# yanyan-li/PlanarSLAM

Measured on AMD Instinct MI355X. Metric: RGB-D frames/sec (extract+match+pose-opt) @640x480; 1->8-GPU batch scaling, higher is better.
Workload: dtype u8/f64

## Files before the change

planarslam_amd/csrc/lsd.hip:

```cpp
#include "common.h"
#include "wave_ops.h"
#include "lsd_nfa.h"
#include "isort.h"

namespace planar {
namespace lsd {

constexpr double LSD_PI = 3.14159265358979323846;
constexpr double M_3_2_PI = 3 * LSD_PI / 2, M_2__PI = 2 * LSD_PI;
constexpr float NOTDEF_F = -1024.0f;
constexpr double DEG_TO_RADS = LSD_PI / 180;
constexpr double RELATIVE_ERROR_FACTOR = 100.0;
constexpr int N_BINS = 1024;
constexpr int MAX_SEGS = 2048;
constexpr int MAX_RECTS = 4096;
constexpr int RING = 512;
constexpr int USED_LDS_BITS = 32768;

struct Plan {
    int W, H, w, h;
    int taps7[7], taps5[5];
    double rho, prec, p, log_nt, density_th, log_eps;
    int min_reg_size;
    size_t off_blur7, off_blur5, off_dx, off_dy, off_ang, off_g2, off_pix, off_seed, off_ord, off_ordr, off_gused, off_tmp, off_reg, off_valid, off_sortr, off_sortb, off_heapj, off_segs, off_kl, off_rects, off_res, off_est, frame_bytes;
    const double* lgamma_tab;
    double p_log[12], p1_log[12], p_log10[12];
    double gaussCoefL[21], gaussCoefG[63];
};

struct Misc { uint32_t g2max; int n_ord; int n_seg; int n_kl; int status; int n_regions; int n_grown_px; int n_rect; long long t[8]; int sort_counts[2]; int heap_n; int sort_kv; int sort_prefix; int pad_; float imp_T; int imp_done; int imp_redo; int imp_full; };

__device__ __forceinline__ float fast_atan2_deg(float y, float x) {
    const float scale = (float)(180 / 3.1415926535897932384626433832795);
    const float p1 = 0.9997878412794807f * scale, p3 = -0.3258083974640975f * scale;
    const float p5 = 0.1555786518463281f * scale, p7 = -0.04432655554792128f * scale;
    const float ax = fabsf(x), ay = fabsf(y);
    float a, c, c2;
    if (ax >= ay) {
        c = ay / (ax + 2.220446049250313e-16f);
        c2 = c * c;
        a = (((p7 * c2 + p5) * c2 + p3) * c2 + p1) * c;
    } else {
        c = ax / (ay + 2.220446049250313e-16f);
        c2 = c * c;
        a = 90.f - (((p7 * c2 + p5) * c2 + p3) * c2 + p1) * c;
    }
    if (x < 0) a = 180.f - a;
    if (y < 0) a = 360.f - a;
    return a;
}

__device__ __forceinline__ int reflect101(int p, int n) {
    if (n == 1) return 0;
    while (p < 0 || p >= n) p = p < 0 ? -p : 2 * n - 2 - p;
    return p;
}

template <int KS>
__global__ __launch_bounds__(256) void lsd_gauss(const uint8_t* __restrict__ src, int pitch, int64_t src_stride, int W, int H,
                                                 const int* __restrict__ taps_g, uint8_t* __restrict__ ws, size_t frame_bytes, size_t off_dst, int B) {
    constexpr int R = KS / 2, TW = 64, TH = 16;
    __shared__ uint8_t s_in[TH + 2 * R][TW + 2 * R];
    __shared__ uint16_t s_h[TH + 2 * R][TW];
    int taps[KS];
    for (int i = 0; i < KS; i++) taps[i] = taps_g[i];
    const int tiles_x = (W + TW - 1) / TW, tiles_y = (H + TH - 1) / TH, tid = threadIdx.x;
    int b, tile;
    xcd_frame_block(tiles_x * tiles_y, B, b, tile);
    const int x0 = (tile % tiles_x) * TW, y0 = (tile / tiles_x) * TH;
    const uint8_t* S = src + (int64_t)b * src_stride;
    for (int i = tid; i < (TH + 2 * R) * (TW + 2 * R); i += 256) {
        const int r = i / (TW + 2 * R), c = i % (TW + 2 * R);
        s_in[r][c] = S[(int64_t)reflect101(y0 + r - R, H) * pitch + reflect101(x0 + c - R, W)];
    }
    __syncthreads();
    for (int i = tid; i < (TH + 2 * R) * TW; i += 256) {
        const int r = i / TW, c = i % TW;
        uint32_t s = 0;
        for (int k = 0; k < KS; k++) s += (uint32_t)taps[k] * s_in[r][c + k];
        s_h[r][c] = (uint16_t)min(s, 65535u);
    }
    __syncthreads();
    uint8_t* D = ws + (size_t)b * frame_bytes + off_dst;
    for (int i = tid; i < TH * TW; i += 256) {
        const int r = i / TW, c = i % TW;
        const int x = x0 + c, y = y0 + r;
        if (x >= W || y >= H) continue;
        uint32_t s = 0;
        for (int k = 0; k < KS; k++) s += (uint32_t)taps[k] * s_h[r + k][c];
        D[(size_t)y * W + x] = (uint8_t)min((s + 32768u) >> 16, 255u);
    }
}

__global__ __launch_bounds__(256) void lsd_gauss75(const uint8_t* __restrict__ src, int pitch, int64_t src_stride, int W, int H, const int* __restrict__ taps_g,
                                                   uint8_t* __restrict__ ws, size_t frame_bytes, size_t off7, size_t off5, int B) {
    constexpr int TW = 64, TH = 16, R = 3, NR = TH + 2 * R, NWD = TW / 4 + 2;
    __shared__ uint32_t s_in[NR][NWD + 1];
    __shared__ __attribute__((aligned(8))) uint16_t s_h7[NR][TW + 4], s_h5[NR][TW + 4];
    int t7[7], t5[5];
    for (int i = 0; i < 7; i++) t7[i] = taps_g[i];
    for (int i = 0; i < 5; i++) t5[i] = taps_g[8 + i];
    const int tiles_x = (W + TW - 1) / TW, tiles_y = (H + TH - 1) / TH, tid = threadIdx.x;
    int b, tile;
    xcd_frame_block(tiles_x * tiles_y, B, b, tile);
    const int x0 = (tile % tiles_x) * TW, y0 = (tile / tiles_x) * TH;
    const uint8_t* S = src + (int64_t)b * src_stride;
    for (int i = tid; i < NR * NWD; i += 256) {
        const int r = i / NWD, wq = i - r * NWD;
        const uint8_t* row = S + (int64_t)reflect101(y0 + r - R, H) * pitch;
        const int xb = x0 - 4 + 4 * wq;
        uint32_t v;
        if (xb >= 0 && xb + 3 < W) v = *(const uint32_t*)(row + xb);
        else v = (uint32_t)row[reflect101(xb, W)] | ((uint32_t)row[reflect101(xb + 1, W)] << 8) | ((uint32_t)row[reflect101(xb + 2, W)] << 16) | ((uint32_t)row[reflect101(xb + 3, W)] << 24);
        s_in[r][wq] = v;
    }
    __syncthreads();
    for (int i = tid; i < NR * (TW / 4); i += 256) {
        const int r = i / (TW / 4), q = i - r * (TW / 4);
        const uint32_t w0 = s_in[r][q], w1 = s_in[r][q + 1], w2 = s_in[r][q + 2];
        uint32_t px[12];
#pragma unroll
        for (int k = 0; k < 4; k++) { px[k] = (w0 >> (8 * k)) & 0xffu; px[4 + k] = (w1 >> (8 * k)) & 0xffu; px[8 + k] = (w2 >> (8 * k)) & 0xffu; }
        uint32_t h7[4], h5[4];
#pragma unroll
        for (int o = 0; o < 4; o++) {
            uint32_t a = 0, c = 0;
#pragma unroll
            for (int k = 0; k < 7; k++) a += (uint32_t)t7[k] * px[o + 1 + k];
#pragma unroll
            for (int k = 0; k < 5; k++) c += (uint32_t)t5[k] * px[o + 2 + k];
            h7[o] = min(a, 65535u); h5[o] = min(c, 65535u);
        }
        *(uint2*)&s_h7[r][4 * q] = make_uint2(h7[0] | (h7[1] << 16), h7[2] | (h7[3] << 16));
        *(uint2*)&s_h5[r][4 * q] = make_uint2(h5[0] | (h5[1] << 16), h5[2] | (h5[3] << 16));
    }
    __syncthreads();
    {
        const int r = tid >> 4, q = tid & 15;
        const int x = x0 + 4 * q, y = y0 + r;
        if (x < W && y < H) {
            uint32_t a[4] = {0, 0, 0, 0}, c[4] = {0, 0, 0, 0};
#pragma unroll
            for (int k = 0; k < 7; k++) {
                const uint2 v = *(const uint2*)&s_h7[r + k][4 * q];
                a[0] += (uint32_t)t7[k] * (v.x & 0xffffu); a[1] += (uint32_t)t7[k] * (v.x >> 16); a[2] += (uint32_t)t7[k] * (v.y & 0xffffu); a[3] += (uint32_t)t7[k] * (v.y >> 16);
            }
#pragma unroll
            for (int k = 0; k < 5; k++) {
                const uint2 v = *(const uint2*)&s_h5[r + 1 + k][4 * q];
                c[0] += (uint32_t)t5[k] * (v.x & 0xffffu); c[1] += (uint32_t)t5[k] * (v.x >> 16); c[2] += (uint32_t)t5[k] * (v.y & 0xffffu); c[3] += (uint32_t)t5[k] * (v.y >> 16);
            }
            uint32_t o7 = 0, o5 = 0;
#pragma unroll
            for (int o = 0; o < 4; o++) { o7 |= min((a[o] + 32768u) >> 16, 255u) << (8 * o); o5 |= min((c[o] + 32768u) >> 16, 255u) << (8 * o); }
            uint8_t* F = ws + (size_t)b * frame_bytes;
            *(uint32_t*)(F + off7 + (size_t)y * W + x) = o7;
            *(uint32_t*)(F + off5 + (size_t)y * W + x) = o5;
        }
    }
}

struct Coef { int ofs, c0, c1; };

__device__ __forceinline__ int scaled_px(const uint8_t* __restrict__ B7, int W, const Coef& cx, const Coef& cy) {
    const uint8_t* r0 = B7 + (size_t)cy.ofs * W + cx.ofs;
    const uint8_t* r1 = r0 + W;
    const uint32_t h0 = min((uint32_t)cx.c0 * r0[0] + (uint32_t)cx.c1 * r0[1], 65535u);
    const uint32_t h1 = min((uint32_t)cx.c0 * r1[0] + (uint32_t)cx.c1 * r1[1], 65535u);
    const uint32_t v = h0 * (uint32_t)cy.c0 + h1 * (uint32_t)cy.c1;
    return (int)min((v + 32768u) >> 16, 255u);
}

__device__ __forceinline__ float2 seed_cos_sin(float deg) {
    const double a = (double)deg * DEG_TO_RADS;
    return make_float2((float)cos(a), (float)sin(a));
}

__global__ __launch_bounds__(256) void lsd_grad(const Plan* __restrict__ plan, const Coef* __restrict__ cxs, const Coef* __restrict__ cys,
                                                uint8_t* __restrict__ ws, Misc* __restrict__ miscs) {
    __shared__ uint8_t s_px[5][68];
    const Plan& P = *plan;
    const int b = blockIdx.z;
    const int x0 = blockIdx.x * 64, y0 = blockIdx.y * 4;
    uint8_t* F = ws + (size_t)b * P.frame_bytes;
    const uint8_t* B7 = F + P.off_blur7;
    for (int i = threadIdx.x; i < 5 * 65; i += 256) {
        const int r = i / 65, c = i - r * 65;
        const int xs = min(x0 + c, P.w - 1), ys = min(y0 + r, P.h - 1);
        s_px[r][c] = (uint8_t)scaled_px(B7, P.W, cxs[xs], cys[ys]);
    }
    __syncthreads();
    const int lx = threadIdx.x & 63, ly = threadIdx.x >> 6;
    const int x = x0 + lx, y = y0 + ly;
    if (x >= P.w || y >= P.h) return;
    float* ang = (float*)(F + P.off_ang);
    uint32_t* g2a = (uint32_t*)(F + P.off_g2);
    float4* pix4 = (float4*)(F + P.off_pix);
    Misc* misc = miscs + b;
    const size_t o = (size_t)y * P.w + x;
    if (x >= P.w - 1 || y >= P.h - 1) { ang[o] = NOTDEF_F; g2a[o] = 0; pix4[o] = make_float4(NOTDEF_F, 0.f, 0.f, 0.f); return; }
    const int s00 = s_px[ly][lx], s10 = s_px[ly][lx + 1], s01 = s_px[ly + 1][lx], s11 = s_px[ly + 1][lx + 1];
    const int DA = s11 - s00, BC = s10 - s01;
    const int gx = DA + BC, gy = DA - BC;
    const int g2 = gx * gx + gy * gy;
    const double norm = sqrt(g2 / 4.0);
    g2a[o] = (uint32_t)g2;
    if (norm <= P.rho) { ang[o] = NOTDEF_F; pix4[o] = make_float4(NOTDEF_F, 0.f, 0.f, 0.f); }
    else {
        const float deg = fast_atan2_deg((float)gx, (float)(-gy));
        ang[o] = deg;
        const double a = (double)deg * DEG_TO_RADS;
        const float af = (float)a;
        pix4[o] = make_float4(deg, (float)cos((double)af), (float)sin((double)af), 0.f);
        atomicMax(&misc->g2max, (uint32_t)g2);
    }
}

template <int NW>
__device__ inline int block_exscan(int v, int* wsum, int* total) {
    const int lane = threadIdx.x & 63, w = threadIdx.x >> 6;
    int inc = v;
    for (int o = 1; o < 64; o <<= 1) { const int t = __shfl_up(inc, o, 64); if (lane >= o) inc += t; }
    __syncthreads();
    if (lane == 63) wsum[w] = inc;
    __syncthreads();
    int base = 0, tot = 0;
    for (int i = 0; i < NW; i++) { if (i < w) base += wsum[i]; tot += wsum[i]; }
    *total = tot;
    return base + inc - v;
}

__device__ __forceinline__ void wave_sync();
__device__ __forceinline__ void lds_sync();
#ifndef PLANAR_WIDE_T
#define PLANAR_WIDE_T 1024
#endif
constexpr int SORT_T = PLANAR_WIDE_T, SORT_LT = 256, SORT_E = 23, SORT_SHIFT = 20, SORT_R = 64;
constexpr int SORT_HJOBS = 1024, SORT_HCAP = 8192, SORT_HY = 2;
using SortLds = isort::LdsLayout<SORT_LT, SORT_E>;
using SortGl = isort::GlobalLayout<SORT_T>;

__global__ __launch_bounds__(SORT_T) void lsd_sort_global(const Plan* __restrict__ plan, uint8_t* __restrict__ ws, Misc* __restrict__ miscs, int rows_cap, int rows_long) {
    extern __shared__ __align__(16) uint8_t sort_lds[];
    __shared__ isort::Range s_init;
    const Plan& P = *plan;
    const int b = blockIdx.x, tid = threadIdx.x, lane = tid & 63;
    uint8_t* F = ws + (size_t)b * P.frame_bytes;
    const uint32_t* g2a = (const uint32_t*)(F + P.off_g2);
    uint32_t* arr = (uint32_t*)(F + P.off_tmp);
    unsigned long long* vb = (unsigned long long*)(F + P.off_valid);
    Misc* misc = miscs + b;
    const int w1 = P.w - 1, h1 = P.h - 1, n = w1 * h1, npix = P.w * P.h;
    const double max_grad = misc->g2max ? sqrt(misc->g2max / 4.0) : -1.0;
    const double bin_coef = (max_grad > 0) ? double(N_BINS - 1) / max_grad : 0;
    const long long ts0 = __builtin_readcyclecounter();
    __shared__ unsigned int s_kv, s_prefix;
    if (tid == 0) { s_kv = 0u; s_prefix = 0u; }
    __syncthreads();
    uint32_t kv = 0;
    for (int p0 = tid - lane; p0 < npix; p0 += SORT_T) {
        const int pix = p0 + lane, y = pix / P.w, x = pix - y * P.w;
        const bool in = pix < npix && x < w1 && y < h1;
        bool valid = false;
        if (in) {
            const double norm = sqrt(g2a[pix] / 4.0);
            const int bin = int(norm * bin_coef);
            arr[pix - y] = ((uint32_t)(N_BINS - 1 - bin) << SORT_SHIFT) | (uint32_t)pix;
            valid = !(norm <= P.rho);
            if (valid) kv = max(kv, (uint32_t)(N_BINS - 1 - bin));
        }
        const unsigned long long m = __ballot(valid);
        if (lane == 0) vb[p0 >> 6] = m;
    }
    kv = (uint32_t)planar::wave_max_f64((double)kv);
    if (lane == 0) atomicMax(&s_kv, kv);
    __syncthreads();
    kv = s_kv;
    int cnt = 0;
    for (int p0 = tid - lane; p0 < npix; p0 += SORT_T) {
        const int pix = p0 + lane, y = pix / P.w, x = pix - y * P.w;
        if (pix < npix && x < w1 && y < h1) cnt += ((arr[pix - y] >> SORT_SHIFT) <= kv) ? 1 : 0;
    }
    cnt = planar::wave_sum_i32(cnt);
    if (lane == 0) atomicAdd(&s_prefix, (unsigned int)cnt);
    if (tid == 0) s_init = isort::Range{0, n, isort::depth_limit(n)};
    __threadfence_block();
    __syncthreads();
    if (tid == 0) { misc->sort_kv = (int)kv; misc->sort_prefix = (int)s_prefix; }
    const isort::HeapSink HS{(isort::HeapJob*)(F + P.off_heapj), &misc->heap_n, SORT_HJOBS};
    isort::global_tier<SORT_SHIFT, SORT_T>(arr, &s_init, 1, SortLds::N, 64, (isort::Range*)(F + P.off_sortr), (isort::Block*)(F + P.off_sortb), isort::G_FMAX,
                                           misc->sort_counts, sort_lds, rows_cap, HS, &misc->status, kv,
                                           rows_long, (uint32_t*)(F + P.off_ord), n / 2 + 1);
    if (tid == 0) misc->t[5] = __builtin_readcyclecounter() - ts0;
}

__global__ __launch_bounds__(SORT_LT, 4) void lsd_sort_lds(const Plan* __restrict__ plan, uint8_t* __restrict__ ws, Misc* __restrict__ miscs) {
    extern __shared__ __align__(16) uint8_t sort_lds[];
    const Plan& P = *plan;
    const int b = blockIdx.x;
    uint8_t* F = ws + (size_t)b * P.frame_bytes;
    Misc* misc = miscs + b;
    const isort::Range* ranges = (const isort::Range*)(F + P.off_sortr);
    const isort::Block* blocks = (const isort::Block*)(F + P.off_sortb);
    const int nb = misc->sort_counts[1];
    const isort::HeapSink HS{(isort::HeapJob*)(F + P.off_heapj), &misc->heap_n, SORT_HJOBS};
    const long long ts0 = __builtin_readcyclecounter();
    for (int k = blockIdx.y; k < nb; k += gridDim.y) {
        const isort::Block K = blocks[k];
        isort::lds_tier<SORT_SHIFT, SORT_LT, SORT_E>((uint32_t*)(F + P.off_tmp), ranges + K.r0, K.nr, K.f, K.l, sort_lds, HS, &misc->status, (uint32_t)misc->sort_kv);
    }
    if (threadIdx.x == 0 && blockIdx.y == 0) misc->t[6] = __builtin_readcyclecounter() - ts0;
}

__global__ __launch_bounds__(64) void lsd_sort_heap(const Plan* __restrict__ plan, uint8_t* __restrict__ ws, Misc* __restrict__ miscs) {
    extern __shared__ __align__(16) uint8_t sort_lds[];
    const Plan& P = *plan;
    uint8_t* F = ws + (size_t)blockIdx.x * P.frame_bytes;
    const int nj = min(miscs[blockIdx.x].heap_n, SORT_HJOBS);
    if (nj) isort::heap_jobs<SORT_SHIFT>((uint32_t*)(F + P.off_tmp), (const isort::HeapJob*)(F + P.off_heapj), nj, blockIdx.y, gridDim.y, (uint32_t*)sort_lds, SORT_HCAP, 0, 1 << 30);
}

__global__ __launch_bounds__(SORT_T) void lsd_sort_compact(const Plan* __restrict__ plan, uint8_t* __restrict__ ws, Misc* __restrict__ miscs) {
    __shared__ int s_cnt[SORT_T / 64];
    const Plan& P = *plan;
    const int b = blockIdx.x, tid = threadIdx.x, lane = tid & 63, wave = tid >> 6;
    uint8_t* F = ws + (size_t)b * P.frame_bytes;
    const uint32_t* arr = (const uint32_t*)(F + P.off_tmp);
    const unsigned long long* vb = (const unsigned long long*)(F + P.off_valid);
    uint32_t* ord = (uint32_t*)(F + P.off_ord);
    uint32_t* ordr = (uint32_t*)(F + P.off_ordr);
    float* pixw = (float*)(F + P.off_pix);
    Misc* misc = miscs + b;
    const int n = min((P.w - 1) * (P.h - 1), misc->sort_prefix);
    const long long ts0 = __builtin_readcyclecounter();
    constexpr int NW = SORT_T / 64, U = 4;
    const int seg = ((n + NW - 1) / NW + 63) & ~63, w0 = min(n, wave * seg), w1 = min(n, w0 + seg);
    auto is_valid = [&](uint32_t e, bool in) { const uint32_t pix = e & 0xfffffu; return in && ((vb[pix >> 6] >> (pix & 63u)) & 1ull); };
    int cnt = 0;
    for (int i0 = w0; i0 < w1; i0 += 64 * U) {
        uint32_t e[U];
#pragma unroll
        for (int u = 0; u < U; u++) e[u] = arr[min(i0 + 64 * u + lane, w1 - 1)];
#pragma unroll
        for (int u = 0; u < U; u++) cnt += __popcll(__ballot(is_valid(e[u], i0 + 64 * u + lane < w1)));
    }
    if (lane == 0) s_cnt[wave] = cnt;
    __syncthreads();
    int pos = 0, total = 0;
    for (int q = 0; q < NW; q++) { if (q < wave) pos += s_cnt[q]; total += s_cnt[q]; }
    for (int i0 = w0; i0 < w1; i0 += 64 * U) {
        uint32_t e[U];
#pragma unroll
        for (int u = 0; u < U; u++) e[u] = arr[min(i0 + 64 * u + lane, w1 - 1)];
#pragma unroll
        for (int u = 0; u < U; u++) {
            const bool v = is_valid(e[u], i0 + 64 * u + lane < w1);
            const unsigned long long m = __ballot(v);
            if (v) {
                const uint32_t pix = e[u] & 0xfffffu, slot = (uint32_t)(pos + __popcll(m & ((1ull << lane) - 1ull)));
                ord[slot] = pix; ordr[slot] = slot;
                pixw[(size_t)pix * 4 + 3] = __uint_as_float(slot);
            }
            pos += __popcll(m);
        }
    }
    if (tid == 0) { misc->n_ord = total; misc->t[7] = __builtin_readcyclecounter() - ts0; }
}

constexpr int SORT_NT = 256, SORT_NW = SORT_NT / 64;
__global__ __launch_bounds__(SORT_NT) void lsd_sort_raster(const Plan* __restrict__ plan, uint8_t* __restrict__ ws, Misc* __restrict__ miscs) {
    __shared__ int wsum[SORT_NW];
    __shared__ int cnt[32 * SORT_NW];
    const Plan& P = *plan;
    const int b = blockIdx.x, tid = threadIdx.x, lane = tid & 63, wave = tid >> 6;
    uint8_t* F = ws + (size_t)b * P.frame_bytes;
    const float* ang = (const float*)(F + P.off_ang);
    const uint32_t* g2a = (const uint32_t*)(F + P.off_g2);
    uint32_t* arr = (uint32_t*)(F + P.off_tmp);
    uint32_t* ord = (uint32_t*)(F + P.off_ord);
    uint32_t* ordr = (uint32_t*)(F + P.off_ordr);
    uint32_t* tmpA = (uint32_t*)(F + P.off_reg);
    Misc* misc = miscs + b;
    const int w1 = P.w - 1, n = w1 * (P.h - 1);
    const double max_grad = misc->g2max ? sqrt(misc->g2max / 4.0) : -1.0;
    const double bin_coef = (max_grad > 0) ? double(N_BINS - 1) / max_grad : 0;
    for (int i = tid; i < n; i += SORT_NT) {
        const int y = i / w1, x = i - y * w1, pix = y * P.w + x;
        arr[i] = ((uint32_t)int(sqrt(g2a[pix] / 4.0) * bin_coef) << 20) | (uint32_t)pix;
    }
    __threadfence_block();
    __syncthreads();
    const long long ts2 = __builtin_readcyclecounter();
    int* wcnt = cnt;
    auto radix_pass = [&](const uint32_t* in, int M, auto digit_of, auto keep, auto emit) -> int {
        const int seg = ((M + SORT_NW - 1) / SORT_NW + 63) & ~63, w0 = min(M, wave * seg), w1 = min(M, w0 + seg);
        for (int t = tid; t < 32 * SORT_NW; t += SORT_NT) wcnt[t] = 0;
        __syncthreads();
        auto match = [&](bool valid, int d) -> unsigned long long {
            unsigned long long same = __ballot(valid);
#pragma unroll
            for (int bit = 0; bit < 5; bit++) { const unsigned long long bm = __ballot(valid && ((d >> bit) & 1)); same &= ((d >> bit) & 1) ? bm : ~bm; }
            return same;
        };
        for (int i0 = w0; i0 < w1; i0 += 64) {
            const int i = i0 + lane;
            const uint32_t e = in[min(i, w1 - 1)];
            const bool valid = i < w1 && keep(e);
            const int d = digit_of(e);
            const unsigned long long same = match(valid, d);
            if (valid && (same & ((1ull << lane) - 1ull)) == 0) wcnt[d * SORT_NW + wave] += __popcll(same);
            lds_sync();
        }
        __syncthreads();
        int total;
        {
            const int v = tid < 32 * SORT_NW ? wcnt[tid] : 0;
            const int ex = block_exscan<SORT_NW>(v, wsum, &total);
            if (tid < 32 * SORT_NW) wcnt[tid] = ex;
        }
        __syncthreads();
        for (int i0 = w0; i0 < w1; i0 += 64) {
            const int i = i0 + lane;
            const uint32_t e = in[min(i, w1 - 1)];
            const bool valid = i < w1 && keep(e);
            const int d = digit_of(e);
            const unsigned long long same = match(valid, d);
            const unsigned long long below = same & ((1ull << lane) - 1ull);
            int base = 0;
            if (valid) base = wcnt[d * SORT_NW + wave];
            lds_sync();
            if (valid) {
                emit(e, i, base + __popcll(below));
                if (below == 0) wcnt[d * SORT_NW + wave] = base + __popcll(same);
            }
            lds_sync();
        }
        __syncthreads();
        return total;
    };
    static_assert(32 * SORT_NW <= SORT_NT, "one thread per radix counter");
    float* pixw = (float*)(F + P.off_pix);
    const int N = radix_pass(arr, n,
        [&](uint32_t e) { return ((N_BINS - 1) - (int)(e >> 20)) & 31; },
        [&](uint32_t e) { return ang[e & 0xfffffu] != NOTDEF_F; },
        [&](uint32_t e, int, int slot) {
            const uint32_t pix = e & 0xfffffu;
            tmpA[slot] = ((uint32_t)((N_BINS - 1) - (int)(e >> 20)) << 20) | pix;
            pixw[(size_t)pix * 4 + 3] = __uint_as_float((uint32_t)slot);
        });
    __threadfence_block();
    __syncthreads();
    radix_pass(tmpA, N,
        [&](uint32_t e) { return (int)((e >> 25) & 31); },
        [&](uint32_t) { return true; },
        [&](uint32_t e, int i, int pos) { ord[pos] = e & 0xfffffu; ordr[pos] = (uint32_t)i; });
    if (tid == 0) { misc->n_ord = N; misc->t[7] = __builtin_readcyclecounter() - ts2; }
}

struct Rect { double x1, y1, x2, y2, width, x, y, theta, dx, dy, prec, p; int pj; };

struct Det {
    const float* ang;
    const uint32_t* g2;
    const float4* pix4;
    const Plan* plan;
    uint32_t* reg;
    uint32_t* tmp;
    int w, h;
    double log_nt;
    uint32_t* used;
    uint32_t* gused;
    uint32_t* ring;
    double* stage;
    int lane;
};

__device__ __forceinline__ bool used_get(const Det& D, uint32_t r) {
    if (r < (uint32_t)USED_LDS_BITS) return (D.used[r >> 5] >> (r & 31)) & 1u;
    return (__hip_atomic_load(D.gused + (r >> 5), __ATOMIC_RELAXED, __HIP_MEMORY_SCOPE_AGENT) >> (r & 31)) & 1u;
}
__device__ __forceinline__ void used_set(const Det& D, uint32_t r) {
    if (r < (uint32_t)USED_LDS_BITS) atomicOr(&D.used[r >> 5], 1u << (r & 31));
    else { atomicOr(D.gused + (r >> 5), 1u << (r & 31)); __builtin_amdgcn_fence(__ATOMIC_SEQ_CST, "agent"); }
}
__device__ __forceinline__ void used_clear(const Det& D, uint32_t r) {
    if (r < (uint32_t)USED_LDS_BITS) atomicAnd(&D.used[r >> 5], ~(1u << (r & 31)));
    else { atomicAnd(D.gused + (r >> 5), ~(1u << (r & 31))); __builtin_amdgcn_fence(__ATOMIC_SEQ_CST, "agent"); }
}
__device__ __forceinline__ uint32_t rank_of(const Det& D, int pix) { return __float_as_uint(D.pix4[pix].w); }
__device__ __forceinline__ double dist2(double x1, double y1, double x2, double y2) { return (x2 - x1) * (x2 - x1) + (y2 - y1) * (y2 - y1); }
__device__ __forceinline__ double angle_diff_signed(double a, double b) {
    double diff = a - b;
    while (diff <= -LSD_PI) diff += M_2__PI;
    while (diff > LSD_PI) diff -= M_2__PI;
    return diff;
}
__device__ __forceinline__ bool aligned_rad(double a, double theta, double prec) {
    double n_theta = theta - a;
    if (n_theta < 0) n_theta = -n_theta;
    if (n_theta > M_3_2_PI) {
        n_theta -= M_2__PI;
        if (n_theta < 0) n_theta = -n_theta;
    }
    return n_theta <= prec;
}
__device__ __forceinline__ void wave_sync() { __builtin_amdgcn_fence(__ATOMIC_SEQ_CST, "workgroup"); __builtin_amdgcn_wave_barrier(); }
__device__ __forceinline__ void lds_sync() { __builtin_amdgcn_fence(__ATOMIC_SEQ_CST, "wavefront"); __builtin_amdgcn_wave_barrier(); }

struct GrowBatch { bool ok; uint32_t nxy; float4 rec4; };
__device__ __forceinline__ GrowBatch grow_fetch(const Det& D, int head, int nb, int reg_n) {
    const int lane = D.lane, w = D.w, h = D.h;
    const int e = lane / 9, k = lane - e * 9;
    GrowBatch g;
    g.ok = false; g.nxy = 0; g.rec4 = make_float4(NOTDEF_F, 0.f, 0.f, 0.f);
    if (lane < 63 && e < nb && k != 4) {
        const int i = head + e;
        uint32_t pxy = D.ring[i & (RING - 1)];
        asm volatile("" : "+v"(pxy));
        if (reg_n - i > RING) pxy = __builtin_nontemporal_load(D.reg + i);
        const int xx = (int)(pxy & 0xffff) + (k % 3) - 1, yy = (int)(pxy >> 16) + (k / 3) - 1;
        if (xx >= 0 && xx < w && yy >= 0 && yy < h) { g.ok = true; g.nxy = (uint32_t)xx | ((uint32_t)yy << 16); g.rec4 = D.pix4[yy * w + xx]; }
    }
    return g;
}
__device__ int region_grow(const Det& D, int seed_pix, uint32_t seed_rank, float seed_deg, float2 seed_cs, double prec, double& reg_angle) {
    const int lane = D.lane;
    reg_angle = (double)seed_deg * DEG_TO_RADS;
    float sumdx = seed_cs.x, sumdy = seed_cs.y;
    const uint32_t seed_xy = (uint32_t)(seed_pix % D.w) | ((uint32_t)(seed_pix / D.w) << 16);
    if (lane == 0) { D.reg[0] = seed_xy; D.ring[0] = seed_xy; used_set(D, seed_rank); }
    lds_sync();
    int reg_n = 1, head = 0, nb = 1;
    GrowBatch cur = grow_fetch(D, 0, 1, 1);
    float4 warm = make_float4(0.f, 0.f, 0.f, 0.f);
    if (lane < 48) {
        const int wy = min(max((int)(seed_xy >> 16) - 8 + lane / 3, 0), D.h - 1), wx = min(max((int)(seed_xy & 0xffff) - 8 + (lane % 3) * 8, 0), D.w - 1);
        warm = D.pix4[wy * D.w + wx];
    }
    while (true) {
        const int head_n = head + nb;
        int nb_n = min(7, reg_n - head_n);
        if (reg_n - head_n > RING) nb_n = 0;
        GrowBatch nxt;
        if (nb_n > 0) nxt = grow_fetch(D, head_n, nb_n, reg_n);
        {
            const float deg = cur.rec4.x, c = cur.rec4.y, sn = cur.rec4.z;
            const uint32_t rk = __float_as_uint(cur.rec4.w);
            bool ok = cur.ok && deg != NOTDEF_F;
            ok = ok && !used_get(D, rk);
            const double a = (double)deg * DEG_TO_RADS;
            int cursor = 0;
            while (true) {
                const bool cand = ok && lane >= cursor && aligned_rad(a, reg_angle, prec);
                const unsigned long long m = __ballot(cand);
                if (!m) break;
                const int f = __builtin_amdgcn_readfirstlane(__ffsll((long long)m) - 1);
                const uint32_t axy = (uint32_t)__builtin_amdgcn_readlane((int)cur.nxy, f);
                const uint32_t ark = (uint32_t)__builtin_amdgcn_readlane((int)rk, f);
                if (lane == 0) { used_set(D, ark); D.reg[reg_n] = axy; D.ring[reg_n & (RING - 1)] = axy; }
                reg_n++;
                sumdx += __int_as_float(__builtin_amdgcn_readlane(__float_as_int(c), f));
                sumdy += __int_as_float(__builtin_amdgcn_readlane(__float_as_int(sn), f));
                reg_angle = (double)fast_atan2_deg(sumdy, sumdx) * DEG_TO_RADS;
                ok = ok && rk != ark;
                cursor = f + 1;
            }
        }
        lds_sync();
        head = head_n;
        if (head >= reg_n) break;
        if (nb_n > 0) { cur = nxt; nb = nb_n; }
        else {
            if (reg_n - head > RING) wave_sync();
            nb = min(7, reg_n - head);
            cur = grow_fetch(D, head, nb, reg_n);
        }
    }
    asm volatile("" :: "v"(warm.x));
    lds_sync();
    return reg_n;
}

template <typename F>
__device__ inline void chains3(const Det& D, int n, double out[3], bool sub2, F vals) {
    const int lane = D.lane;
    double acc = 0;
    for (int base = 0; base < n; base += 64) {
        const int i = base + lane;
        if (i < n) { double v[3]; vals(i, v); D.stage[lane * 3] = v[0]; D.stage[lane * 3 + 1] = v[1]; D.stage[lane * 3 + 2] = v[2]; }
        lds_sync();
        const int cnt = min(64, n - base);
        if (lane < 3) {
            const double* st = D.stage + lane;
            const bool neg = lane == 2 && sub2;
            int j = 0;
            for (; j + 8 <= cnt; j += 8) {
                double v[8];
#pragma unroll
                for (int u = 0; u < 8; u++) v[u] = st[(j + u) * 3];
#pragma unroll
                for (int u = 0; u < 8; u++) { if (neg) acc -= v[u]; else acc += v[u]; }
            }
            for (; j < cnt; j++) { if (neg) acc -= st[j * 3]; else acc += st[j * 3]; }
        }
        lds_sync();
    }
    out[0] = planar::wave_lane(acc, 0); out[1] = planar::wave_lane(acc, 1); out[2] = planar::wave_lane(acc, 2);
}

__device__ inline double wave_max_d(double v) { return planar::wave_max_f64(v); }
__device__ inline double wave_min_d(double v) { return planar::wave_min_f64(v); }
__device__ inline int wave_sum_i(int v) { return planar::wave_sum_i32(v); }

__device__ __forceinline__ double modgrad_of(const Det& D, uint32_t pxy) { return sqrt(D.g2[(pxy >> 16) * D.w + (pxy & 0xffff)] / 4.0); }

__device__ void region2rect(const Det& D, int n, double reg_angle, double prec, double p, Rect& rec) {
    double s3[3];
    chains3(D, n, s3, false, [&](int i, double* v) {
        const uint32_t e = D.reg[i];
        const double wgt = modgrad_of(D, e);
        v[0] = double(e & 0xffff) * wgt; v[1] = double(e >> 16) * wgt; v[2] = wgt;
    });
    const double x = s3[0] / s3[2], y = s3[1] / s3[2];
    chains3(D, n, s3, true, [&](int i, double* v) {
        const uint32_t e = D.reg[i];
        const double wgt = modgrad_of(D, e);
        const double dx = double(e & 0xffff) - x, dy = double(e >> 16) - y;
        v[0] = dy * dy * wgt; v[1] = dx * dx * wgt; v[2] = dx * dy * wgt;
    });
    const double Ixx = s3[0], Iyy = s3[1], Ixy = s3[2];
    const double lambda = 0.5 * (Ixx + Iyy - sqrt((Ixx - Iyy) * (Ixx - Iyy) + 4.0 * Ixy * Ixy));
    double theta = (fabs(Ixx) > fabs(Iyy)) ? double(fast_atan2_deg(float(lambda - Ixx), float(Ixy))) : double(fast_atan2_deg(float(Ixy), float(lambda - Iyy)));
    theta *= DEG_TO_RADS;
    if (fabs(angle_diff_signed(theta, reg_angle)) > prec) theta += LSD_PI;
    const double dx = cos(theta), dy = sin(theta);
    double l_min = 0, l_max = 0, w_min = 0, w_max = 0;
    for (int i = D.lane; i < n; i += 64) {
        const uint32_t e = D.reg[i];
        const double regdx = double(e & 0xffff) - x, regdy = double(e >> 16) - y;
        const double l = regdx * dx + regdy * dy;
        const double w = -regdx * dy + regdy * dx;
        l_max = fmax(l_max, l); l_min = fmin(l_min, l); w_max = fmax(w_max, w); w_min = fmin(w_min, w);
    }
    l_max = wave_max_d(l_max); l_min = wave_min_d(l_min); w_max = wave_max_d(w_max); w_min = wave_min_d(w_min);
    rec.x1 = x + l_min * dx; rec.y1 = y + l_min * dy;
    rec.x2 = x + l_max * dx; rec.y2 = y + l_max * dy;
    rec.width = w_max - w_min;
    rec.x = x; rec.y = y; rec.theta = theta; rec.dx = dx; rec.dy = dy; rec.prec = prec; rec.p = p; rec.pj = 0;
    if (rec.width < 1.0) rec.width = 1.0;
}

__device__ bool reduce_region_radius(const Det& D, int& n, double reg_angle, double prec, double p, Rect& rec, double density, double density_th) {
    const int lane = D.lane;
    const uint32_t e0 = D.reg[0];
    const double xc = double(e0 & 0xffff), yc = double(e0 >> 16);
    const double radSq1 = dist2(xc, yc, rec.x1, rec.y1), radSq2 = dist2(xc, yc, rec.x2, rec.y2);
    double radSq = radSq1 > radSq2 ? radSq1 : radSq2;
    while (density < density_th) {
        radSq *= 0.75 * 0.75;
        int n_near = 0;
        for (int i = lane; i < n; i += 64) {
            const uint32_t e = D.reg[i];
            const bool far = dist2(xc, yc, double(e & 0xffff), double(e >> 16)) > radSq;
            if (far) used_clear(D, rank_of(D, (e >> 16) * D.w + (e & 0xffff)));
            else n_near++;
        }
        n_near = wave_sum_i(n_near);
        int k = 0;
        for (int base = n - 1; base >= n_near; base -= 64) {
            const int pos = base - lane;
            bool near = false;
            uint32_t e = 0;
            if (pos >= n_near) { e = D.reg[pos]; near = !(dist2(xc, yc, double(e & 0xffff), double(e >> 16)) > radSq); }
            const unsigned long long m = __ballot(near);
            if (near) D.tmp[k + __popcll(m & ((1ull << lane) - 1))] = e;
            k += __popcll(m);
        }
        wave_sync();
        k = 0;
        for (int base = 0; base < n_near; base += 64) {
            const int pos = base + lane;
            bool far = false;
            if (pos < n_near) { const uint32_t e = D.reg[pos]; far = dist2(xc, yc, double(e & 0xffff), double(e >> 16)) > radSq; }
            const unsigned long long m = __ballot(far);
            if (far) D.reg[pos] = D.tmp[k + __popcll(m & ((1ull << lane) - 1))];
            k += __popcll(m);
        }
        wave_sync();
        n = n_near;
        if (n < 2) return false;
        region2rect(D, n, reg_angle, prec, p, rec);
        density = double(n) / (sqrt(dist2(rec.x1, rec.y1, rec.x2, rec.y2)) * rec.width);
    }
    return true;
}

__device__ bool refine(const Det& D, int& n, double& reg_angle, double prec, double p, Rect& rec, double density_th) {
    double density = double(n) / (sqrt(dist2(rec.x1, rec.y1, rec.x2, rec.y2)) * rec.width);
    if (density >= density_th) return true;
    const uint32_t e0 = D.reg[0];
    const double xc = double(e0 & 0xffff), yc = double(e0 >> 16);
    const int seed_pix = (e0 >> 16) * D.w + (e0 & 0xffff);
    const double ang_c = (double)D.ang[seed_pix] * DEG_TO_RADS;
    const double width = rec.width;
    double s3[3];
    int cnt = 0;
    chains3(D, n, s3, false, [&](int i, double* v) {
        const uint32_t e = D.reg[i];
        const int pix = (e >> 16) * D.w + (e & 0xffff);
        used_clear(D, rank_of(D, pix));
        v[0] = 0; v[1] = 0; v[2] = 0;
        if (sqrt(dist2(xc, yc, double(e & 0xffff), double(e >> 16))) < width) {
            const double ang_d = angle_diff_signed((double)D.ang[pix] * DEG_TO_RADS, ang_c);
            v[0] = ang_d; v[1] = ang_d * ang_d; cnt++;
        }
    });
    cnt = wave_sum_i(cnt);
    const double sum = s3[0], s_sum = s3[1];
    const double mean_angle = sum / double(cnt);
    const double tau = 2.0 * sqrt((s_sum - 2.0 * mean_angle * sum) / double(cnt) + mean_angle * mean_angle);
    wave_sync();
    n = region_grow(D, seed_pix, rank_of(D, seed_pix), D.ang[seed_pix], seed_cos_sin(D.ang[seed_pix]), tau, reg_angle);
    wave_sync();
    if (n < 2) return false;
    region2rect(D, n, reg_angle, prec, p, rec);
    density = double(n) / (sqrt(dist2(rec.x1, rec.y1, rec.x2, rec.y2)) * rec.width);
    if (density < density_th) return reduce_region_radius(D, n, reg_angle, prec, p, rec, density, density_th);
    return true;
}

__device__ inline bool double_equal(double a, double b) {
    if (a == b) return true;
    const double abs_diff = fabs(a - b), aa = fabs(a), bb = fabs(b);
    double abs_max = (aa > bb) ? aa : bb;
    if (abs_max < 2.2250738585072014e-308) abs_max = 2.2250738585072014e-308;
    return (abs_diff / abs_max) <= (RELATIVE_ERROR_FACTOR * 2.220446049250313e-16);
}
__device__ double nfa(const Plan& P, int n, int k, double p, int pj, int lane, double beat = -1.7976931348623157e308) {
    const double LOG_NT = P.log_nt;
    if (n == 0 || k == 0) return -LOG_NT;
    if (n == k) return -LOG_NT - double(n) * P.p_log10[pj];
    const double p_term = p / (1 - p);
    const double* lg = P.lgamma_tab;
    const double log1term = lg[n + 1] - lg[k + 1] - lg[n - k + 1] + double(k) * P.p_log[pj] + double(n - k) * P.p1_log[pj];
    {
        const double bound = -log1term / 2.30258509299404568402 - LOG_NT;
        if (bound < beat - 1e-9 * (1.0 + fabs(beat) + fabs(bound))) return bound;
    }
    double term = exp(log1term);
    if (double_equal(term, 0)) {
        if (k > n * p) return -log1term / 2.30258509299404568402 - LOG_NT;
        else return -LOG_NT;
    }
    return nfa_tail(term, n, k, p_term, LOG_NT, lane);
}

template <int NP>
__device__ int rect_counts(const Det& D, const Rect& rec, const double* precs, int* alg_out) {
    const int lane = D.lane;
    const double half_width = rec.width / 2.0;
    const double dyhw = rec.dy * half_width, dxhw = rec.dx * half_width;
    int ox[4], oy[4];
    ox[0] = int(rec.x1 - dyhw); oy[0] = int(rec.y1 + dxhw);
    ox[1] = int(rec.x2 - dyhw); oy[1] = int(rec.y2 + dxhw);
    ox[2] = int(rec.x2 + dyhw); oy[2] = int(rec.y2 - dxhw);
    ox[3] = int(rec.x1 + dyhw); oy[3] = int(rec.y1 - dxhw);
    for (int i = 1; i < 4; i++) {
        const int vx = ox[i], vy = oy[i];
        int j = i - 1;
        while (j >= 0 && (vx == ox[j] ? vy < oy[j] : vx < ox[j])) { ox[j + 1] = ox[j]; oy[j + 1] = oy[j]; j--; }
        ox[j + 1] = vx; oy[j + 1] = vy;
    }
    int min_y = 0, max_y = 0;
    for (int i = 1; i < 4; ++i) {
        if (oy[min_y] > oy[i]) min_y = i;
        if (oy[max_y] < oy[i]) max_y = i;
    }
    bool taken[4] = {false, false, false, false};
    taken[min_y] = true;
    int leftmost = -1;
    for (int i = 0; i < 4; ++i) if (!taken[i]) { if (leftmost < 0) leftmost = i; else if (ox[leftmost] > ox[i]) leftmost = i; }
    taken[leftmost] = true;
    int rightmost = -1;
    for (int i = 0; i < 4; ++i) if (!taken[i]) { if (rightmost < 0) rightmost = i; else if (ox[rightmost] < ox[i]) rightmost = i; }
    taken[rightmost] = true;
    int tailp = -1;
    for (int i = 0; i < 4; ++i) if (!taken[i]) { if (tailp < 0) tailp = i; else if (ox[tailp] > ox[i]) tailp = i; }
    const long long flstep = (oy[min_y] != oy[leftmost]) ? (ox[min_y] - ox[leftmost]) / (oy[min_y] - oy[leftmost]) : 0;
    const long long slstep = (oy[leftmost] != ox[tailp]) ? (ox[leftmost] - ox[tailp]) / (oy[leftmost] - ox[tailp]) : 0;
    const long long frstep = (oy[min_y] != oy[rightmost]) ? (ox[min_y] - ox[rightmost]) / (oy[min_y] - oy[rightmost]) : 0;
    const long long srstep = (oy[rightmost] != ox[tailp]) ? (ox[rightmost] - ox[tailp]) / (oy[rightmost] - ox[tailp]) : 0;
    const long long x0 = ox[min_y];
    const int ylo = max(oy[min_y], 0), yhi = min(oy[max_y], D.h - 1);
    const int nrows = yhi >= ylo ? yhi - ylo + 1 : 0;
    const int ly = oy[leftmost], ry = oy[rightmost];
    auto row_span = [&](int k, int& xa) -> int {
        const long long nl = min(max((long long)ly - ylo, 0ll), (long long)k), nr = min(max((long long)ry - ylo, 0ll), (long long)k);
        const long long left = x0 + nl * flstep + (k - nl) * slstep, right = x0 + nr * frstep + (k - nr) * srstep;
        const long long a = max(left, 0ll), b = min(right, (long long)D.w - 1);
        xa = (int)a;
        return b >= a ? (int)(b - a + 1) : 0;
    };
    int total = 0, wmax = 0;
    for (int k = lane; k < nrows; k += 64) { int xa; const int c = row_span(k, xa); total += c; wmax = max(wmax, c); }
    total = wave_sum_i(total);
    wmax = (int)planar::wave_max_f64((double)wmax);
    int alg[NP];
    for (int q = 0; q < NP; q++) alg[q] = 0;
    auto test = [&](float deg) {
        if (deg == NOTDEF_F) return;
        double n_theta = rec.theta - (double)deg * DEG_TO_RADS;
        if (n_theta < 0) n_theta = -n_theta;
        if (n_theta > M_3_2_PI) {
            n_theta -= M_2__PI;
            if (n_theta < 0) n_theta = -n_theta;
        }
        for (int q = 0; q < NP; q++) if (n_theta <= precs[q]) alg[q]++;
    };
    constexpr int RU = 4;
    if (wmax > 0 && wmax <= 64) {
        int wp = 1; while (wp < wmax) wp <<= 1;
        const int rps = 64 / wp, sub = lane / wp, xo = lane & (wp - 1);
        for (int kb = 0; kb < nrows; kb += rps * RU) {
            int pix[RU]; float deg[RU];
#pragma unroll
            for (int u = 0; u < RU; u++) {
                const int k = kb + u * rps + sub;
                pix[u] = -1;
                if (k < nrows) { int xa; const int c = row_span(k, xa); if (xo < c) pix[u] = (ylo + k) * D.w + xa + xo; }
            }
#pragma unroll
            for (int u = 0; u < RU; u++) deg[u] = D.ang[max(pix[u], 0)];
#pragma unroll
            for (int u = 0; u < RU; u++) if (pix[u] >= 0) test(deg[u]);
        }
    } else if (wmax > 64) {
        for (int k = 0; k < nrows; k++) {
            int xa; const int c = row_span(k, xa);
            const int base = (ylo + k) * D.w + xa;
            for (int x0 = 0; x0 < c; x0 += 64 * RU) {
                float deg[RU];
#pragma unroll
                for (int u = 0; u < RU; u++) deg[u] = D.ang[base + min(x0 + 64 * u + lane, c - 1)];
#pragma unroll
                for (int u = 0; u < RU; u++) if (x0 + 64 * u + lane < c) test(deg[u]);
            }
        }
    }
    for (int q = 0; q < NP; q++) alg_out[q] = wave_sum_i(alg[q]);
    return total;
}

__device__ double rect_nfa(const Det& D, const Rect& rec, double beat) {
    int alg;
    const int total = rect_counts<1>(D, rec, &rec.prec, &alg);
    return nfa(*D.plan, total, alg, rec.p, rec.pj, D.lane, beat);
}

__device__ double rect_improve(const Det& D, Rect& rec, double LOG_EPS) {
    const double delta = 0.5, delta_2 = delta / 2.0;
    const Plan& P = *D.plan;
    Rect r = rec;
    double precs[6], ps[6];
    precs[0] = rec.prec; ps[0] = rec.p;
    for (int n = 1; n < 6; ++n) { ps[n] = ps[n - 1] / 2; precs[n] = ps[n] * LSD_PI; }
    int algs[6];
    const int total0 = rect_counts<6>(D, rec, precs, algs);
    double log_nfa = nfa(P, total0, algs[0], ps[0], rec.pj, D.lane);
    if (log_nfa > LOG_EPS) return log_nfa;
    for (int n = 0; n < 5; ++n) {
        r.p /= 2;
        r.prec = r.p * LSD_PI;
        r.pj++;
        const double v = nfa(P, total0, algs[n + 1], r.p, r.pj, D.lane, log_nfa);
        if (v > log_nfa) { log_nfa = v; rec = r; }
    }
    if (log_nfa > LOG_EPS) return log_nfa;
    r = rec;
    for (int n = 0; n < 5; ++n) {
        if ((r.width - delta) >= 0.5) {
            r.width -= delta;
            const double v = rect_nfa(D, r, log_nfa);
            if (v > log_nfa) { rec = r; log_nfa = v; }
        }
    }
// ... 902 lines not shown
```

Before: 12430.

## Speculatively commit multiple aligned neighbors per wave step in LSD region growing

Region growing moves into a header and gains a speculative batch-commit path. When several lanes are aligned candidates, prefix sums of the gradient vectors give each lane the region angle it would see. The wave then re-checks alignment and commits the longest prefix that agrees with the serial order, instead of adding one pixel per ballot iteration. Duplicate neighbors shared between batch elements are masked so the serial semantics hold. This adds prefix-sum, duplicate-mask and extra ballot overhead, and the floating-point summation order may differ slightly from the serial path.

```diff
diff --git a/planarslam_amd/csrc/lsd.hip b/planarslam_amd/csrc/lsd.hip
--- a/planarslam_amd/csrc/lsd.hip
+++ b/planarslam_amd/csrc/lsd.hip
@@ -1,21 +1,16 @@
 #include "common.h"
 #include "wave_ops.h"
 #include "lsd_nfa.h"
+#include "lsd_grow.h"
 #include "isort.h"
 
 namespace planar {
 namespace lsd {
 
-constexpr double LSD_PI = 3.14159265358979323846;
-constexpr double M_3_2_PI = 3 * LSD_PI / 2, M_2__PI = 2 * LSD_PI;
-constexpr float NOTDEF_F = -1024.0f;
-constexpr double DEG_TO_RADS = LSD_PI / 180;
 constexpr double RELATIVE_ERROR_FACTOR = 100.0;
 constexpr int N_BINS = 1024;
 constexpr int MAX_SEGS = 2048;
 constexpr int MAX_RECTS = 4096;
-constexpr int RING = 512;
-constexpr int USED_LDS_BITS = 32768;
 
 struct Plan {
     int W, H, w, h;
@@ -29,26 +24,6 @@
 };
 
 struct Misc { uint32_t g2max; int n_ord; int n_seg; int n_kl; int status; int n_regions; int n_grown_px; int n_rect; long long t[8]; int sort_counts[2]; int heap_n; int sort_kv; int sort_prefix; int pad_; float imp_T; int imp_done; int imp_redo; int imp_full; };
-
-__device__ __forceinline__ float fast_atan2_deg(float y, float x) {
-    const float scale = (float)(180 / 3.1415926535897932384626433832795);
-    const float p1 = 0.9997878412794807f * scale, p3 = -0.3258083974640975f * scale;
-    const float p5 = 0.1555786518463281f * scale, p7 = -0.04432655554792128f * scale;
-    const float ax = fabsf(x), ay = fabsf(y);
-    float a, c, c2;
-    if (ax >= ay) {
-        c = ay / (ax + 2.220446049250313e-16f);
-        c2 = c * c;
-        a = (((p7 * c2 + p5) * c2 + p3) * c2 + p1) * c;
-    } else {
-        c = ax / (ay + 2.220446049250313e-16f);
-        c2 = c * c;
-        a = 90.f - (((p7 * c2 + p5) * c2 + p3) * c2 + p1) * c;
-    }
-    if (x < 0) a = 180.f - a;
-    if (y < 0) a = 360.f - a;
-    return a;
-}
 
 __device__ __forceinline__ int reflect101(int p, int n) {
     if (n == 1) return 0;
@@ -230,8 +205,6 @@
     return base + inc - v;
 }
 
-__device__ __forceinline__ void wave_sync();
-__device__ __forceinline__ void lds_sync();
 #ifndef PLANAR_WIDE_T
 #define PLANAR_WIDE_T 1024
 #endif
@@ -459,34 +432,6 @@
 
 struct Rect { double x1, y1, x2, y2, width, x, y, theta, dx, dy, prec, p; int pj; };
 
-struct Det {
-    const float* ang;
-    const uint32_t* g2;
-    const float4* pix4;
-    const Plan* plan;
-    uint32_t* reg;
-    uint32_t* tmp;
-    int w, h;
-    double log_nt;
-    uint32_t* used;
-    uint32_t* gused;
-    uint32_t* ring;
-    double* stage;
-    int lane;
-};
-
-__device__ __forceinline__ bool used_get(const Det& D, uint32_t r) {
-    if (r < (uint32_t)USED_LDS_BITS) return (D.used[r >> 5] >> (r & 31)) & 1u;
-    return (__hip_atomic_load(D.gused + (r >> 5), __ATOMIC_RELAXED, __HIP_MEMORY_SCOPE_AGENT) >> (r & 31)) & 1u;
-}
-__device__ __forceinline__ void used_set(const Det& D, uint32_t r) {
-    if (r < (uint32_t)USED_LDS_BITS) atomicOr(&D.used[r >> 5], 1u << (r & 31));
-    else { atomicOr(D.gused + (r >> 5), 1u << (r & 31)); __builtin_amdgcn_fence(__ATOMIC_SEQ_CST, "agent"); }
-}
-__device__ __forceinline__ void used_clear(const Det& D, uint32_t r) {
-    if (r < (uint32_t)USED_LDS_BITS) atomicAnd(&D.used[r >> 5], ~(1u << (r & 31)));
-    else { atomicAnd(D.gused + (r >> 5), ~(1u << (r & 31))); __builtin_amdgcn_fence(__ATOMIC_SEQ_CST, "agent"); }
-}
 __device__ __forceinline__ uint32_t rank_of(const Det& D, int pix) { return __float_as_uint(D.pix4[pix].w); }
 __device__ __forceinline__ double dist2(double x1, double y1, double x2, double y2) { return (x2 - x1) * (x2 - x1) + (y2 - y1) * (y2 - y1); }
 __device__ __forceinline__ double angle_diff_signed(double a, double b) {
@@ -495,92 +440,6 @@
     while (diff > LSD_PI) diff -= M_2__PI;
     return diff;
 }
-__device__ __forceinline__ bool aligned_rad(double a, double theta, double prec) {
-    double n_theta = theta - a;
-    if (n_theta < 0) n_theta = -n_theta;
-    if (n_theta > M_3_2_PI) {
-        n_theta -= M_2__PI;
-        if (n_theta < 0) n_theta = -n_theta;
-    }
-    return n_theta <= prec;
-}
-__device__ __forceinline__ void wave_sync() { __builtin_amdgcn_fence(__ATOMIC_SEQ_CST, "workgroup"); __builtin_amdgcn_wave_barrier(); }
-__device__ __forceinline__ void lds_sync() { __builtin_amdgcn_fence(__ATOMIC_SEQ_CST, "wavefront"); __builtin_amdgcn_wave_barrier(); }
-
-struct GrowBatch { bool ok; uint32_t nxy; float4 rec4; };
-__device__ __forceinline__ GrowBatch grow_fetch(const Det& D, int head, int nb, int reg_n) {
-    const int lane = D.lane, w = D.w, h = D.h;
-    const int e = lane / 9, k = lane - e * 9;
-    GrowBatch g;
-    g.ok = false; g.nxy = 0; g.rec4 = make_float4(NOTDEF_F, 0.f, 0.f, 0.f);
-    if (lane < 63 && e < nb && k != 4) {
-        const int i = head + e;
-        uint32_t pxy = D.ring[i & (RING - 1)];
-        asm volatile("" : "+v"(pxy));
-        if (reg_n - i > RING) pxy = __builtin_nontemporal_load(D.reg + i);
-        const int xx = (int)(pxy & 0xffff) + (k % 3) - 1, yy = (int)(pxy >> 16) + (k / 3) - 1;
-        if (xx >= 0 && xx < w && yy >= 0 && yy < h) { g.ok = true; g.nxy = (uint32_t)xx | ((uint32_t)yy << 16); g.rec4 = D.pix4[yy * w + xx]; }
-    }
-    return g;
-}
-__device__ int region_grow(const Det& D, int seed_pix, uint32_t seed_rank, float seed_deg, float2 seed_cs, double prec, double& reg_angle) {
-    const int lane = D.lane;
-    reg_angle = (double)seed_deg * DEG_TO_RADS;
-    float sumdx = seed_cs.x, sumdy = seed_cs.y;
-    const uint32_t seed_xy = (uint32_t)(seed_pix % D.w) | ((uint32_t)(seed_pix / D.w) << 16);
-    if (lane == 0) { D.reg[0] = seed_xy; D.ring[0] = seed_xy; used_set(D, seed_rank); }
-    lds_sync();
-    int reg_n = 1, head = 0, nb = 1;
-    GrowBatch cur = grow_fetch(D, 0, 1, 1);
-    float4 warm = make_float4(0.f, 0.f, 0.f, 0.f);
-    if (lane < 48) {
-        const int wy = min(max((int)(seed_xy >> 16) - 8 + lane / 3, 0), D.h - 1), wx = min(max((int)(seed_xy & 0xffff) - 8 + (lane % 3) * 8, 0), D.w - 1);
-        warm = D.pix4[wy * D.w + wx];
-    }
-    while (true) {
-        const int head_n = head + nb;
-        int nb_n = min(7, reg_n - head_n);
-        if (reg_n - head_n > RING) nb_n = 0;
-        GrowBatch nxt;
-        if (nb_n > 0) nxt = grow_fetch(D, head_n, nb_n, reg_n);
-        {
-            const float deg = cur.rec4.x, c = cur.rec4.y, sn = cur.rec4.z;
-            const uint32_t rk = __float_as_uint(cur.rec4.w);
-            bool ok = cur.ok && deg != NOTDEF_F;
-            ok = ok && !used_get(D, rk);
-            const double a = (double)deg * DEG_TO_RADS;
-            int cursor = 0;
-            while (true) {
-                const bool cand = ok && lane >= cursor && aligned_rad(a, reg_angle, prec);
-                const unsigned long long m = __ballot(cand);
-                if (!m) break;
-                const int f = __builtin_amdgcn_readfirstlane(__ffsll((long long)m) - 1);
-                const uint32_t axy = (uint32_t)__builtin_amdgcn_readlane((int)cur.nxy, f);
-                const uint32_t ark = (uint32_t)__builtin_amdgcn_readlane((int)rk, f);
-                if (lane == 0) { used_set(D, ark); D.reg[reg_n] = axy; D.ring[reg_n & (RING - 1)] = axy; }
-                reg_n++;
-                sumdx += __int_as_float(__builtin_amdgcn_readlane(__float_as_int(c), f));
-                sumdy += __int_as_float(__builtin_amdgcn_readlane(__float_as_int(sn), f));
-                reg_angle = (double)fast_atan2_deg(sumdy, sumdx) * DEG_TO_RADS;
-                ok = ok && rk != ark;
-                cursor = f + 1;
-            }
-        }
-        lds_sync();
-        head = head_n;
-        if (head >= reg_n) break;
-        if (nb_n > 0) { cur = nxt; nb = nb_n; }
-        else {
-            if (reg_n - head > RING) wave_sync();
-            nb = min(7, reg_n - head);
-            cur = grow_fetch(D, head, nb, reg_n);
-        }
-    }
-    asm volatile("" :: "v"(warm.x));
-    lds_sync();
-    return reg_n;
-}
-
 template <typename F>
 __device__ inline void chains3(const Det& D, int n, double out[3], bool sub2, F vals) {
     const int lane = D.lane;
diff --git a/planarslam_amd/csrc/lsd_grow.h b/planarslam_amd/csrc/lsd_grow.h
--- /dev/null
+++ b/planarslam_amd/csrc/lsd_grow.h
@@ -0,0 +1,206 @@
+#pragma once
+#include "wave_ops.h"
+
+#ifdef PLANAR_WAVE_EMUL
+#define LSD_OPAQUE_V(x) ((void)0)
+#define LSD_KEEP_V(x) ((void)(x))
+#else
+#define LSD_OPAQUE_V(x) asm volatile("" : "+v"(x))
+#define LSD_KEEP_V(x) asm volatile("" ::"v"(x))
+#endif
+
+namespace planar {
+namespace lsd {
+
+constexpr double LSD_PI = 3.14159265358979323846;
+constexpr double M_3_2_PI = 3 * LSD_PI / 2, M_2__PI = 2 * LSD_PI;
+constexpr float NOTDEF_F = -1024.0f;
+constexpr double DEG_TO_RADS = LSD_PI / 180;
+constexpr int RING = 512;
+constexpr int USED_LDS_BITS = 32768;
+
+struct Plan;
+
+__device__ __forceinline__ float fast_atan2_deg(float y, float x) {
+    const float scale = (float)(180 / 3.1415926535897932384626433832795);
+    const float p1 = 0.9997878412794807f * scale, p3 = -0.3258083974640975f * scale;
+    const float p5 = 0.1555786518463281f * scale, p7 = -0.04432655554792128f * scale;
+    const float ax = fabsf(x), ay = fabsf(y);
+    float a, c, c2;
+    if (ax >= ay) {
+        c = ay / (ax + 2.220446049250313e-16f);
+        c2 = c * c;
+        a = (((p7 * c2 + p5) * c2 + p3) * c2 + p1) * c;
+    } else {
+        c = ax / (ay + 2.220446049250313e-16f);
+        c2 = c * c;
+        a = 90.f - (((p7 * c2 + p5) * c2 + p3) * c2 + p1) * c;
+    }
+    if (x < 0) a = 180.f - a;
+    if (y < 0) a = 360.f - a;
+    return a;
+}
+
+struct Det {
+    const float* ang;
+    const uint32_t* g2;
+    const float4* pix4;
+    const Plan* plan;
+    uint32_t* reg;
+    uint32_t* tmp;
+    int w, h;
+    double log_nt;
+    uint32_t* used;
+    uint32_t* gused;
+    uint32_t* ring;
+    double* stage;
+    int lane;
+};
+
+__device__ __forceinline__ bool used_get(const Det& D, uint32_t r) {
+    if (r < (uint32_t)USED_LDS_BITS) return (D.used[r >> 5] >> (r & 31)) & 1u;
+    return (__hip_atomic_load(D.gused + (r >> 5), __ATOMIC_RELAXED, __HIP_MEMORY_SCOPE_AGENT) >> (r & 31)) & 1u;
+}
+__device__ __forceinline__ void used_set(const Det& D, uint32_t r) {
+    if (r < (uint32_t)USED_LDS_BITS) atomicOr(&D.used[r >> 5], 1u << (r & 31));
+    else { atomicOr(D.gused + (r >> 5), 1u << (r & 31)); __builtin_amdgcn_fence(__ATOMIC_SEQ_CST, "agent"); }
+}
+__device__ __forceinline__ void used_clear(const Det& D, uint32_t r) {
+    if (r < (uint32_t)USED_LDS_BITS) atomicAnd(&D.used[r >> 5], ~(1u << (r & 31)));
+    else { atomicAnd(D.gused + (r >> 5), ~(1u << (r & 31))); __builtin_amdgcn_fence(__ATOMIC_SEQ_CST, "agent"); }
+}
+__device__ __forceinline__ bool aligned_rad(double a, double theta, double prec) {
+    double n_theta = theta - a;
+    if (n_theta < 0) n_theta = -n_theta;
+    if (n_theta > M_3_2_PI) {
+        n_theta -= M_2__PI;
+        if (n_theta < 0) n_theta = -n_theta;
+    }
+    return n_theta <= prec;
+}
+__device__ __forceinline__ int lanes_below(unsigned long long m) {
+#ifdef PLANAR_WAVE_EMUL
+    return __popcll(m & ((1ull << (threadIdx.x & 63)) - 1ull));
+#else
+    return (int)__builtin_amdgcn_mbcnt_hi((unsigned)(m >> 32), __builtin_amdgcn_mbcnt_lo((unsigned)m, 0u));
+#endif
+}
+__device__ __forceinline__ void wave_sync() { __builtin_amdgcn_fence(__ATOMIC_SEQ_CST, "workgroup"); __builtin_amdgcn_wave_barrier(); }
+__device__ __forceinline__ void lds_sync() { __builtin_amdgcn_fence(__ATOMIC_SEQ_CST, "wavefront"); __builtin_amdgcn_wave_barrier(); }
+
+struct GrowBatch { bool ok; uint32_t nxy; float4 rec4; };
+__device__ __forceinline__ GrowBatch grow_fetch(const Det& D, int head, int nb, int reg_n) {
+    const int lane = D.lane, w = D.w, h = D.h;
+    const int e = lane / 9, k = lane - e * 9;
+    GrowBatch g;
+    g.ok = false; g.nxy = 0; g.rec4 = make_float4(NOTDEF_F, 0.f, 0.f, 0.f);
+    if (lane < 63 && e < nb) {
+        const int i = head + e;
+        uint32_t pxy = D.ring[i & (RING - 1)];
+        LSD_OPAQUE_V(pxy);
+        if (reg_n - i > RING) pxy = __builtin_nontemporal_load(D.reg + i);
+        const int xx = (int)(pxy & 0xffff) + (k % 3) - 1, yy = (int)(pxy >> 16) + (k / 3) - 1;
+        if (k == 4) g.nxy = pxy;
+        else if (xx >= 0 && xx < w && yy >= 0 && yy < h) { g.ok = true; g.nxy = (uint32_t)xx | ((uint32_t)yy << 16); g.rec4 = D.pix4[yy * w + xx]; }
+    }
+    return g;
+}
+
+__device__ int region_grow(const Det& D, int seed_pix, uint32_t seed_rank, float seed_deg, float2 seed_cs, double prec, double& reg_angle) {
+    const int lane = D.lane;
+    reg_angle = (double)seed_deg * DEG_TO_RADS;
+    float sumdx = seed_cs.x, sumdy = seed_cs.y;
+    const uint32_t seed_xy = (uint32_t)(seed_pix % D.w) | ((uint32_t)(seed_pix / D.w) << 16);
+    if (lane == 0) { D.reg[0] = seed_xy; D.ring[0] = seed_xy; used_set(D, seed_rank); }
+    lds_sync();
+    int reg_n = 1, head = 0, nb = 1;
+    GrowBatch cur = grow_fetch(D, 0, 1, 1);
+    float4 warm = make_float4(0.f, 0.f, 0.f, 0.f);
+    if (lane < 48) {
+        const int wy = min(max((int)(seed_xy >> 16) - 8 + lane / 3, 0), D.h - 1), wx = min(max((int)(seed_xy & 0xffff) - 8 + (lane % 3) * 8, 0), D.w - 1);
+        warm = D.pix4[wy * D.w + wx];
+    }
+    while (true) {
+        const int head_n = head + nb;
+        int nb_n = min(7, reg_n - head_n);
+        if (reg_n - head_n > RING) nb_n = 0;
+        GrowBatch nxt;
+        if (nb_n > 0) nxt = grow_fetch(D, head_n, nb_n, reg_n);
+        {
+            const float deg = cur.rec4.x, c = cur.rec4.y, sn = cur.rec4.z;
+            const uint32_t rk = __float_as_uint(cur.rec4.w);
+            bool ok = cur.ok && deg != NOTDEF_F;
+            ok = ok && !used_get(D, rk);
+            const double a = (double)deg * DEG_TO_RADS;
+            int cursor = 0;
+            bool dup_ready = false;
+            unsigned long long dupm = 0;
+            while (true) {
+                const bool cand = ok && lane >= cursor && aligned_rad(a, reg_angle, prec);
+                const unsigned long long m0 = __ballot(cand);
+                if (!m0) break;
+                if ((m0 & (m0 - 1ull)) == 0ull) {
+                    const int f = __builtin_amdgcn_readfirstlane(__ffsll((long long)m0) - 1);
+                    const uint32_t ark = (uint32_t)__builtin_amdgcn_readlane((int)rk, f);
+                    if (lane == f) { used_set(D, ark); D.reg[reg_n] = cur.nxy; D.ring[reg_n & (RING - 1)] = cur.nxy; }
+                    reg_n++;
+                    sumdx += __int_as_float(__builtin_amdgcn_readlane(__float_as_int(c), f));
+                    sumdy += __int_as_float(__builtin_amdgcn_readlane(__float_as_int(sn), f));
+                    reg_angle = (double)fast_atan2_deg(sumdy, sumdx) * DEG_TO_RADS;
+                    ok = ok && rk != ark;
+                    cursor = f + 1;
+                    continue;
+                }
+                if (!dup_ready) {
+                    const int e = lane / 9, px = (int)(cur.nxy & 0xffff), py = (int)(cur.nxy >> 16);
+                    for (int q = 0; q + 1 < nb; q++) {
+                        const uint32_t exy = (uint32_t)__builtin_amdgcn_readlane((int)cur.nxy, q * 9 + 4);
+                        const int dx = px - (int)(exy & 0xffff) + 1, dy = py - (int)(exy >> 16) + 1;
+                        if (q < e && (unsigned)dx < 3u && (unsigned)dy < 3u) dupm |= 1ull << (q * 9 + dy * 3 + dx);
+                    }
+                    dup_ready = true;
+                }
+                const bool spec = cand && (dupm & m0) == 0ull;
+                const unsigned long long m = __ballot(spec);
+                float ux = sumdx, uy = sumdy, px = sumdx, py = sumdy;
+                for (unsigned long long mm = m; mm; mm &= mm - 1ull) {
+                    const int j = __builtin_amdgcn_readfirstlane(__ffsll((long long)mm) - 1);
+                    ux += __int_as_float(__builtin_amdgcn_readlane(__float_as_int(c), j));
+                    uy += __int_as_float(__builtin_amdgcn_readlane(__float_as_int(sn), j));
+                    if (lane > j) { px = ux; py = uy; }
+                }
+                const double th = lanes_below(m) ? (double)fast_atan2_deg(py, px) * DEG_TO_RADS : reg_angle;
+                const bool dec = ok && lane >= cursor && (dupm & m) == 0ull && aligned_rad(a, th, prec);
+                const unsigned long long x = __ballot(dec != spec);
+                const int mpos = x ? __builtin_amdgcn_readfirstlane(__ffsll((long long)x) - 1) : 64;
+                const unsigned long long commit = mpos < 64 ? m & ((1ull << mpos) - 1ull) : m;
+                if ((commit >> lane) & 1ull) {
+                    const int slot = reg_n + lanes_below(commit);
+                    used_set(D, rk); D.reg[slot] = cur.nxy; D.ring[slot & (RING - 1)] = cur.nxy;
+                }
+                reg_n += __popcll(commit);
+                const int src = min(mpos, 63);
+                sumdx = __int_as_float(__builtin_amdgcn_readlane(__float_as_int(px), src));
+                sumdy = __int_as_float(__builtin_amdgcn_readlane(__float_as_int(py), src));
+                reg_angle = planar::wave_lane(th, src);
+                ok = ok && (dupm & commit) == 0ull;
+                cursor = mpos;
+            }
+        }
+        lds_sync();
+        head = head_n;
+        if (head >= reg_n) break;
+        if (nb_n > 0) { cur = nxt; nb = nb_n; }
+        else {
+            if (reg_n - head > RING) wave_sync();
+            nb = min(7, reg_n - head);
+            cur = grow_fetch(D, head, nb, reg_n);
+        }
+    }
+    LSD_KEEP_V(warm.x);
+    lds_sync();
+    return reg_n;
+}
+
+}
+}
```

Result: no change. 12530 (median of 6 runs) (+0.8%).
